# hbell99/DirectVoxGO

Hardware: AMD Instinct MI355X
Metric: train rays/sec (8192-ray batch, 160^3 grid) (higher is better)
Workload: dtype f32

## Files before the change

### directvoxgo_amd/csrc/common.h

```cpp
#pragma once
#include <hip/hip_runtime.h>
#include <stdint.h>

#include "../../include/dvgo_hip.h"

#define DVGO_WAVE 64
#define DVGO_BLOCK 256

#define DVGO_LAUNCH_CHECK()                                   \
  do {                                                        \
    hipError_t e__ = hipGetLastError();                       \
    if (e__ != hipSuccess) return (int)e__;                   \
  } while (0)

#define DVGO_HIP_TRY(expr)                                    \
  do {                                                        \
    hipError_t e__ = (expr);                                  \
    if (e__ != hipSuccess) return (int)e__;                   \
  } while (0)

static inline int dvgo_blocks(int64_t work, int per_block) {
  return (int)((work + per_block - 1) / per_block);
}

static inline bool dvgo_fits(int64_t work) { return work >= 0 && work < ((int64_t)1 << 31); }

__device__ __forceinline__ float dvgo_relu(float z) { return __builtin_elementwise_maximum(z, 0.0f); }
__device__ __forceinline__ unsigned int dvgo_relu_bit(float r) { return __float_as_uint(r) != 0u ? 1u : 0u; }

struct TriSetup {
  int i0, j0, k0;
  float wx0, wx1, wy0, wy1, wz0, wz1;
  float gx, gy, gz;
};

__device__ __forceinline__ float dvgo_src_index(float p, float mn, float mx, int size) {
  const float u = (p - mn) / (mx - mn);
  const float c = u * 2.0f - 1.0f;
  return ((c + 1.0f) / 2.0f) * (float)(size - 1);
}

__device__ __forceinline__ TriSetup dvgo_tri_from_g(float gx, float gy, float gz) {
  TriSetup t;
  const float fx = floorf(gx), fy = floorf(gy), fz = floorf(gz);
  t.i0 = (int)fx; t.j0 = (int)fy; t.k0 = (int)fz;
  t.wx0 = (fx + 1.0f) - gx; t.wx1 = gx - fx;
  t.wy0 = (fy + 1.0f) - gy; t.wy1 = gy - fy;
  t.wz0 = (fz + 1.0f) - gz; t.wz1 = gz - fz;
  t.gx = gx; t.gy = gy; t.gz = gz;
  return t;
}

__device__ __forceinline__ TriSetup dvgo_tri_setup(float px, float py, float pz,
                                                   float mnx, float mny, float mnz,
                                                   float mxx, float mxy, float mxz,
                                                   int X, int Y, int Z) {
  const float gx = dvgo_src_index(px, mnx, mxx, X);
  const float gy = dvgo_src_index(py, mny, mxy, Y);
  const float gz = dvgo_src_index(pz, mnz, mxz, Z);
  return dvgo_tri_from_g(gx, gy, gz);
}
// ... 144 lines not shown
```

### directvoxgo_amd/csrc/loss.hip

```cpp
#include "common.h"

__device__ __forceinline__ float block_sum_256(float v, float* red) {
#pragma unroll
  for (int d = 32; d >= 1; d >>= 1) v += __shfl_xor(v, d);
  const int lane = threadIdx.x & 63, w = threadIdx.x >> 6;
  if (lane == 0) red[w] = v;
  __syncthreads();
  const float t = red[0] + red[1] + red[2] + red[3];
  __syncthreads();
  return t;
}

__global__ void __launch_bounds__(256)
loss_rays_kernel(const float* __restrict__ rgb_marched, const float* __restrict__ alphainv_last,
                 const float* __restrict__ target, int64_t N, float inv_n_global, float w_main, float w_ent,
                 float* __restrict__ g_marched, float* __restrict__ g_last, float* __restrict__ loss_out) {
  __shared__ float red[4];
  const int64_t r = (int64_t)blockIdx.x * blockDim.x + threadIdx.x;
  float l = 0.0f;
  if (r < N) {
    float se = 0.0f;
#pragma unroll
    for (int c = 0; c < 3; ++c) {
      const float d = rgb_marched[3 * r + c] - target[3 * r + c];
// ... 5 lines not shown
      const float x = alphainv_last[r];
      const float p = fminf(fmaxf(x, 1e-6f), 1.0f - 1e-6f);
      const float lp = logf(p), lq = logf(1.0f - p);
      l += w_ent * (-(p * lp + (1.0f - p) * lq)) * inv_n_global;
      const bool inside = (x >= 1e-6f) && (x <= 1.0f - 1e-6f);
      g_last[r] = inside ? w_ent * (lq - lp) * inv_n_global : 0.0f;
    } else {
      g_last[r] = 0.0f;
    }
  }
  const float t = block_sum_256(l, red);
  if (threadIdx.x == 0) atomicAdd(loss_out, t);
}

__global__ void __launch_bounds__(256)
loss_samples_kernel(const float* __restrict__ raw_rgb, const float* __restrict__ weights,
                    const int64_t* __restrict__ ray_id, const float* __restrict__ target, int64_t M_cap,
                    const int64_t* __restrict__ m_dev,
                    float inv_n_global, float w_per, float* __restrict__ g_raw_rgb, float* __restrict__ loss_out) {
  const int64_t M = m_dev ? (*m_dev < M_cap ? *m_dev : M_cap) : M_cap;
  __shared__ float red[4];
  float l = 0.0f;
  for (int64_t i = (int64_t)blockIdx.x * blockDim.x + threadIdx.x; i < M; i += (int64_t)gridDim.x * blockDim.x) {
    const int64_t r = ray_id[i];
    const float w = weights[i];
    float se = 0.0f;
#pragma unroll
    for (int c = 0; c < 3; ++c) {
      const float d = raw_rgb[3 * i + c] - target[3 * r + c];
      se = fmaf(d, d, se);
      g_raw_rgb[3 * i + c] = 2.0f * w_per * w * d * inv_n_global;
    }
    l += w_per * w * se * inv_n_global;
  }
  const float t = block_sum_256(l, red);
  if (threadIdx.x == 0) atomicAdd(loss_out, t);
}

__global__ void __launch_bounds__(256)
viewdir_embed_kernel(const float* __restrict__ viewdirs, const float* __restrict__ freq, int F, int64_t N,
                     float* __restrict__ emb) {
  const int E = 3 + 6 * F;
  const int64_t t = (int64_t)blockIdx.x * blockDim.x + threadIdx.x;
  if (t >= N * E) return;
  const int64_t r = t / E;
  const int e = (int)(t - r * E);
  float v;
  if (e < 3) v = viewdirs[3 * r + e];
  else {
    const int q = (e - 3) % (3 * F);
    const float a = viewdirs[3 * r + q / F] * freq[q % F];
    v = (e - 3 < 3 * F) ? sinf(a) : cosf(a);
  }
  emb[t] = v;
}

#define DVGO_MT_MAX 16
struct AdamMulti {
  float* p[DVGO_MT_MAX];
  const float* g[DVGO_MT_MAX];
  float* m[DVGO_MT_MAX];
  float* v[DVGO_MT_MAX];
  int64_t start[DVGO_MT_MAX + 1];
  int n;
};
__global__ void __launch_bounds__(256)
// ... 44 lines not shown
  for (int k = n_tensors; k <= 8; ++k) A.start[k] = tot;
  if (tot == 0) return 0;
  if (!dvgo_fits(tot)) return DVGO_ERANGE;
  copy_multi_kernel<<<dvgo_blocks(tot, 256), 256, 0, (hipStream_t)stream>>>(A);
  DVGO_LAUNCH_CHECK();
  return 0;
}

int dvgo_loss_fwd_bwd(const float* rgb_marched, const float* alphainv_last, const float* target, int64_t N,
                      const float* raw_rgb, const float* weights, const int64_t* ray_id, int64_t M, const int64_t* m_dev,
                      int64_t n_rays_global, float w_main, float w_ent, float w_per, float* g_marched,
                      float* g_last, float* g_raw_rgb, float* loss_out, void* stream) {
  if (N < 0 || M < 0 || n_rays_global <= 0) return DVGO_EINVAL;
  if (!loss_out) return DVGO_EINVAL;
  hipStream_t s = (hipStream_t)stream;
  DVGO_HIP_TRY(hipMemsetAsync(loss_out, 0, sizeof(float), s));
  const float inv = 1.0f / (float)n_rays_global;
  if (N > 0) {
    if (!rgb_marched || !alphainv_last || !target || !g_marched || !g_last) return DVGO_EINVAL;
    loss_rays_kernel<<<dvgo_blocks(N, 256), 256, 0, s>>>(rgb_marched, alphainv_last, target, N, inv, w_main, w_ent,
                                                         g_marched, g_last, loss_out);
    DVGO_LAUNCH_CHECK();
  }
  if (M > 0 && w_per > 0.0f) {
    if (!raw_rgb || !weights || !ray_id || !g_raw_rgb) return DVGO_EINVAL;
    const int64_t nb = dvgo_blocks(M, 256);
    loss_samples_kernel<<<(int)(nb < 256 ? nb : (M >= (1 << 20) ? 1024 : 256)), 256, 0, s>>>(raw_rgb, weights, ray_id, target, M, m_dev, inv, w_per,
                                                            g_raw_rgb, loss_out);
    DVGO_LAUNCH_CHECK();
  }
  return 0;
}

int dvgo_viewdir_embed(const float* viewdirs, const float* freq, int n_freq, int64_t N, float* emb, void* stream) {
  if (N < 0 || n_freq < 0) return DVGO_EINVAL;
  if (N == 0) return 0;
  if (!viewdirs || !emb || (n_freq > 0 && !freq)) return DVGO_EINVAL;
  const int64_t total = N * (3 + 6 * n_freq);
  if (!dvgo_fits(total)) return DVGO_ERANGE;
  viewdir_embed_kernel<<<dvgo_blocks(total, 256), 256, 0, (hipStream_t)stream>>>(viewdirs, freq, n_freq, N, emb);
  DVGO_LAUNCH_CHECK();
  return 0;
}

int dvgo_adam_upd_multi(float* const* params, const float* const* grads, float* const* exp_avg,
                        float* const* exp_avg_sq, const int64_t* numel, int n_tensors, float step_size, float beta1,
                        float beta2, float eps, const float* step_size_dev, void* stream) {
  if (n_tensors < 0 || n_tensors > DVGO_MT_MAX) return DVGO_EINVAL;
  if (n_tensors == 0) return 0;
  if (!params || !grads || !exp_avg || !exp_avg_sq || !numel) return DVGO_EINVAL;
  AdamMulti A;
  A.n = n_tensors;
  int64_t tot = 0;
  for (int k = 0; k < n_tensors; ++k) {
    if (numel[k] < 0 || (numel[k] > 0 && (!params[k] || !grads[k] || !exp_avg[k] || !exp_avg_sq[k]))) return DVGO_EINVAL;
    A.p[k] = params[k]; A.g[k] = grads[k]; A.m[k] = exp_avg[k]; A.v[k] = exp_avg_sq[k];
    A.start[k] = tot;
    tot += numel[k];
  }
  for (int k = n_tensors; k <= DVGO_MT_MAX; ++k) A.start[k] = tot;
  if (tot == 0) return 0;
  adam_multi_kernel<<<dvgo_blocks(tot, 256), 256, 0, (hipStream_t)stream>>>(A, step_size, step_size_dev, beta1, beta2, eps);
  DVGO_LAUNCH_CHECK();
  return 0;
}

// ... 2 lines not shown
```

### directvoxgo_amd/csrc/shade_x3.hip

```cpp
#include "common.h"
#include "x3.h"

#ifndef X3_THREADS
#define X3_THREADS 512
#endif
#define X3_WAVES (X3_THREADS / 64)
#ifndef X3_BWD_THREADS
#define X3_BWD_THREADS 512
#endif
#define X3_BWD_WAVES (X3_BWD_THREADS / 64)
#define X3_STAGE_ROWS 16
#define X3_STAGE_STRIDE 36

__device__ __forceinline__ int x3_acc_feature(int t, int r, int h) { return 32 * t + (r & 3) + 8 * (r >> 2) + 4 * h; }

__device__ __forceinline__ void x3_split1(float v, unsigned short& s0, unsigned short& s1, unsigned short& s2) {
  const unsigned int h = x3_pack(v, 0.f) & 0xffffu;
  const float r = v - __uint_as_float(h << 16);
  const unsigned int m = x3_pack(r, 0.f) & 0xffffu;
  const float q = r - __uint_as_float(m << 16);
  s0 = (unsigned short)h; s1 = (unsigned short)m; s2 = (unsigned short)(x3_pack(q, 0.f) & 0xffffu);
}

template <int WIDTH, int KS1>
// ... 52 lines not shown
  for (int i = tid; i < T * KS1 * 64 * 8; i += nt) {
    const int j = i & 7, l = (i >> 3) & 63, s = (i >> 9) % KS1, t = (i >> 9) / KS1;
    const int k = 16 * s + 8 * (l >> 5) + j;
    const float v = (k < D_in) ? W1[(32 * t + (l & 31)) * D_in + k] : 0.0f;
    unsigned short p0, p1, p2;
    x3_split1(v, p0, p1, p2);
    reinterpret_cast<unsigned short*>(&L.w1s[t][s][0][l])[j] = p0;
    reinterpret_cast<unsigned short*>(&L.w1s[t][s][1][l])[j] = p1;
    reinterpret_cast<unsigned short*>(&L.w1s[t][s][2][l])[j] = p2;
  }
  for (int i = tid; i < T * 2 * T * 64 * 8; i += nt) {
    const int j = i & 7, l = (i >> 3) & 63, ks = (i >> 9) % (2 * T), t2 = (i >> 9) / (2 * T);
    const int k = 16 * ks + 8 * (j >> 2) + 4 * (l >> 5) + (j & 3);
    const float v = W2[(32 * t2 + (l & 31)) * WIDTH + k];
    unsigned short p0, p1, p2;
    x3_split1(v, p0, p1, p2);
    reinterpret_cast<unsigned short*>(&L.w2s[t2][ks][0][l])[j] = p0;
    reinterpret_cast<unsigned short*>(&L.w2s[t2][ks][1][l])[j] = p1;
    reinterpret_cast<unsigned short*>(&L.w2s[t2][ks][2][l])[j] = p2;
  }
  for (int i = tid; i < 3 * 2 * T * 16; i += nt) {
    const int tr = i % (T * 16), h = (i / (T * 16)) & 1, c = i / (2 * T * 16);
    (&L.w3p[0][0][0])[i] = W3[c * WIDTH + x3_acc_feature(tr >> 4, tr & 15, h)];
  }
  for (int i = tid; i < 2 * T * 16; i += nt) {
    const int tr = i % (T * 16), h = i / (T * 16);
    const int f = x3_acc_feature(tr >> 4, tr & 15, h);
    (&L.b1p[0][0])[i] = b1[f];
    (&L.b2p[0][0])[i] = b2[f];
  }
  if (tid < 4) L.b3[tid] = tid < 3 ? b3[tid] : 0.0f;
}

template <int WIDTH, int KS1, bool DIFFUSE>
__global__ void __launch_bounds__(X3_THREADS)
shade_fwd_x3_kernel(const float* __restrict__ feat, int C, int c_view0, int n_view, const float* __restrict__ emb, int E,
                    const int64_t* __restrict__ ray_id, int64_t M_cap, const int64_t* __restrict__ m_dev,
                    const void* __restrict__ image, float* __restrict__ rgb,
                    float* __restrict__ H1, float* __restrict__ H2, unsigned long long* __restrict__ masks, int experiment) {
  const int64_t M = m_dev ? (*m_dev < M_cap ? *m_dev : M_cap) : M_cap;
  constexpr int T = WIDTH / 32;
  __shared__ __attribute__((aligned(16))) X3Lds<WIDTH, KS1> L;
  x3_copy_image<X3Img<WIDTH, KS1>>(&L, image);
  __syncthreads();
  const int lane = threadIdx.x & 63, h = lane >> 5;
  float* stage = L.stage[threadIdx.x >> 6];
  const bool train = H1 != nullptr;
  const int64_t n_tiles = (M + 31) / 32;
  const int64_t gw = (int64_t)blockIdx.x * (blockDim.x >> 6) + (threadIdx.x >> 6);
  const int64_t nw = (int64_t)gridDim.x * (blockDim.x >> 6);
  const int d_in = n_view + E;
  const int64_t last = M > 0 ? M - 1 : 0;
  auto row_of = [&](int64_t tile) { const int64_t r = tile * 32 + (lane & 31); return r < M ? r : last; };
  float xin[KS1][8];
  auto load_inputs = [&](int64_t tile, int64_t rid) {
    const float* fr = feat + row_of(tile) * C + c_view0;
    const float* er = emb + rid * E - n_view;
#pragma unroll
    for (int s = 0; s < KS1; ++s)
#pragma unroll
      for (int j = 0; j < 8; ++j) {
        const int k = 16 * s + 8 * h + j;
        const int kc = k < d_in ? k : d_in - 1;
        xin[s][j] = *((kc < n_view) ? fr + kc : er + kc);
      }
  };
  int64_t rid_n = 0;
  if (gw < n_tiles) { load_inputs(gw, ray_id[row_of(gw)]); rid_n = ray_id[row_of(gw + nw)]; }
  for (int64_t tile = gw; tile < n_tiles; tile += nw) {
    const int64_t row = tile * 32 + (lane & 31);
    const bool valid = row < M;
    const int rows_valid = (int)(M - tile * 32 < 32 ? M - tile * 32 : 32);
    u32x4 x3[KS1][3];
#pragma unroll
    for (int s = 0; s < KS1; ++s) {
      float v[8];
#pragma unroll
      for (int j = 0; j < 8; ++j) v[j] = (16 * s + 8 * h + j) < d_in ? xin[s][j] : 0.0f;
      x3_split8(v, x3[s][0], x3[s][1], x3[s][2]);
    }
    load_inputs(tile + nw, rid_n);
    rid_n = ray_id[row_of(tile + 2 * nw)];
    u32x4 h3[2 * T][3];
    unsigned long long mask1 = 0ull;
#pragma unroll
    for (int t = 0; t < T; ++t) {
      f32x16 acc;
#pragma unroll
      for (int r = 0; r < 16; ++r) acc[r] = L.b1p[h][t * 16 + r];
#pragma unroll
      for (int s = 0; s < KS1; ++s)
        x3_mfma6(acc, L.w1s[t][s][0][lane], L.w1s[t][s][1][lane], L.w1s[t][s][2][lane], x3[s][0], x3[s][1], x3[s][2]);
#pragma unroll
      for (int r = 0; r < 16; ++r) acc[r] = dvgo_relu(acc[r]);
      if (train) {
        unsigned int bits = 0u;
#pragma unroll
        for (int r = 0; r < 16; ++r) bits |= dvgo_relu_bit(acc[r]) << r;
        mask1 |= (unsigned long long)bits << (16 * t);
        if (!(experiment & 512)) x3_store_tile(stage, acc, H1 + tile * 32 * WIDTH + 32 * t, WIDTH, lane, rows_valid);
      }
#pragma unroll
      for (int s2 = 0; s2 < 2; ++s2) {
        float v[8];
#pragma unroll
        for (int j = 0; j < 8; ++j) v[j] = acc[8 * s2 + j];
        x3_split8(v, h3[2 * t + s2][0], h3[2 * t + s2][1], h3[2 * t + s2][2]);
      }
      __builtin_amdgcn_sched_barrier(0);
    }
    float p[3] = {0.0f, 0.0f, 0.0f};
    unsigned long long mask2 = 0ull;
#pragma unroll 1
    for (int t2 = 0; t2 < T; ++t2) {
      f32x16 acc2;
#pragma unroll
      for (int r = 0; r < 16; ++r) acc2[r] = L.b2p[h][t2 * 16 + r];
      u32x4 a[2][3];
#pragma unroll
      for (int q = 0; q < 3; ++q) a[0][q] = L.w2s[t2][0][q][lane];
#pragma unroll
      for (int ks = 0; ks < 2 * T; ++ks) {
        if (ks + 1 < 2 * T) {
#pragma unroll
          for (int q = 0; q < 3; ++q) a[(ks + 1) & 1][q] = L.w2s[t2][ks + 1][q][lane];
        }
        x3_mfma6(acc2, a[ks & 1][0], a[ks & 1][1], a[ks & 1][2], h3[ks][0], h3[ks][1], h3[ks][2]);
        __builtin_amdgcn_sched_barrier(0);
      }
#pragma unroll
      for (int r = 0; r < 16; ++r) acc2[r] = dvgo_relu(acc2[r]);
      if (train) {
        unsigned int bits = 0u;
#pragma unroll
        for (int r = 0; r < 16; ++r) bits |= dvgo_relu_bit(acc2[r]) << r;
        mask2 |= (unsigned long long)bits << (16 * t2);
        if (!(experiment & 512)) x3_store_tile(stage, acc2, H2 + tile * 32 * WIDTH + 32 * t2, WIDTH, lane, rows_valid);
      }
#pragma unroll
      for (int c = 0; c < 3; ++c) {
#pragma unroll
        for (int r = 0; r < 16; ++r) p[c] = fmaf(L.w3p[c][h][t2 * 16 + r], acc2[r], p[c]);
      }
    }
    float z[3];
#pragma unroll
    for (int c = 0; c < 3; ++c) z[c] = p[c] + __shfl_xor(p[c], 32) + L.b3[c];
    if (valid) {
      if (h == 0) {
#pragma unroll
        for (int c = 0; c < 3; ++c) {
          const float zz = DIFFUSE ? z[c] + feat[row * C + c] : z[c];
          rgb[row * 3 + c] = 1.0f / (1.0f + expf(-zz));
        }
      }
      if (train) {
        masks[(row * 2 + 0) * 2 + h] = mask1;
        masks[(row * 2 + 1) * 2 + h] = mask2;
      }
    }
  }
}

template <int WIDTH>
struct X3BwdImg {
  static constexpr int T = WIDTH / 32;
  u32x4 w2t[T][2 * T][3][64];
  u32x4 w1t[2 * T][3][64];
// ... 853 lines not shown
}

extern "C" {

int64_t dvgo_shade_scratch_bytes(int width) {
  if (width == 128) return (int64_t)sizeof(X3Img<128, 3>) > (int64_t)sizeof(X3BwdImg<128>) ? sizeof(X3Img<128, 3>) : sizeof(X3BwdImg<128>);
  if (width == 64) return (int64_t)sizeof(X3Img<64, 3>) > (int64_t)sizeof(X3BwdImg<64>) ? sizeof(X3Img<64, 3>) : sizeof(X3BwdImg<64>);
  return 0;
}

int dvgo_shade_fwd_x3(const float* feat, int C, const float* emb, int E, const int64_t* ray_id, int64_t M, const int64_t* m_dev,
                      const float* W1, const float* b1, const float* W2, const float* b2, const float* W3,
                      const float* b3, int width, int d_in, int diffuse, float* rgb, float* H1, float* H2,
                      uint64_t* masks, void* scratch, void* scratch_bwd, int experiment, void* stream) {
  if (M < 0 || C <= 0 || E < 0) return DVGO_EINVAL;
  if (M == 0) return 0;
  if (!feat || !emb || !ray_id || !W1 || !b1 || !W2 || !b2 || !W3 || !b3 || !rgb || !scratch) return DVGO_EINVAL;
  if ((H1 == nullptr) != (H2 == nullptr) || (H1 == nullptr) != (masks == nullptr)) return DVGO_EINVAL;
  const int c_view0 = diffuse ? 3 : 0;
  const int n_view = C - c_view0;
  if (n_view < 0 || d_in != n_view + E) return DVGO_EINVAL;
  if ((width != 128 && width != 64) || d_in > 48) return DVGO_ERANGE;
  hipStream_t s = (hipStream_t)stream;
  const int64_t n_tiles = (M + 31) / 32;
  const int64_t cap = 256;
  const int blocks = (int)((n_tiles + X3_WAVES - 1) / X3_WAVES < cap ? (n_tiles + X3_WAVES - 1) / X3_WAVES : cap);
#define DVGO_SHADE_X3(W, KS, DIFF)                                                                                       \
  do {                                                                                                                   \
    x3_prep_fwd_kernel<W, KS><<<scratch_bwd ? 64 : 32, 256, 0, s>>>((X3Img<W, KS>*)scratch, (X3BwdImg<W>*)scratch_bwd, W1, b1, W2, b2, W3, b3, d_in); \
    shade_fwd_x3_kernel<W, KS, DIFF><<<blocks, X3_THREADS, 0, s>>>(feat, C, c_view0, n_view, emb, E, ray_id, M, m_dev, scratch, rgb, \
                                                                    H1, H2, (unsigned long long*)masks, experiment);     \
  } while (0)
  if (width == 128) {
    if (diffuse) DVGO_SHADE_X3(128, 3, true); else DVGO_SHADE_X3(128, 3, false);
  } else {
    if (d_in <= 16) { if (diffuse) DVGO_SHADE_X3(64, 1, true); else DVGO_SHADE_X3(64, 1, false); }
    else            { if (diffuse) DVGO_SHADE_X3(64, 3, true); else DVGO_SHADE_X3(64, 3, false); }
  }
#undef DVGO_SHADE_X3
  DVGO_LAUNCH_CHECK();
  return 0;
}

int dvgo_shade_bwd_x3(const float* g_rgb, const float* rgb, const uint64_t* masks, int64_t M, const int64_t* m_dev,
                      const float* W1, const float* W2, const float* W3, int width, int d_in, int C, int diffuse,
                      float* g_feat, float* G1, float* gz, void* scratch, int prebuilt, void* stream) {
  if (M < 0 || C <= 0) return DVGO_EINVAL;
  if (M == 0) return 0;
  if (!g_rgb || !rgb || !masks || !W1 || !W2 || !W3 || !g_feat || !G1 || !gz || !scratch) return DVGO_EINVAL;
  const int c_view0 = diffuse ? 3 : 0;
  const int n_view = C - c_view0;
  if ((width != 128 && width != 64) || n_view < 0 || n_view > 32 || d_in < n_view) return DVGO_ERANGE;
  hipStream_t s = (hipStream_t)stream;
  const int64_t n_tiles = (M + 31) / 32;
  const int64_t cap = 256;
  const int blocks = (int)((n_tiles + X3_BWD_WAVES - 1) / X3_BWD_WAVES < cap ? (n_tiles + X3_BWD_WAVES - 1) / X3_BWD_WAVES : cap);
#define DVGO_SHADE_BWD_X3(W, DIFF)                                                                                        \
  do {                                                                                                                    \
    if (!prebuilt) x3_prep_bwd_kernel<W><<<32, 256, 0, s>>>((X3BwdImg<W>*)scratch, W1, W2, W3, d_in);                   \
    shade_bwd_x3_kernel<W, DIFF><<<blocks, X3_BWD_THREADS, 0, s>>>(g_rgb, rgb, (const unsigned long long*)masks, M, m_dev, scratch, C, \
                                                                c_view0, n_view, g_feat, G1, gz);                         \
  } while (0)
  if (width == 128) { if (diffuse) DVGO_SHADE_BWD_X3(128, true); else DVGO_SHADE_BWD_X3(128, false); }
  else              { if (diffuse) DVGO_SHADE_BWD_X3(64, true); else DVGO_SHADE_BWD_X3(64, false); }
#undef DVGO_SHADE_BWD_X3
  DVGO_LAUNCH_CHECK();
  return 0;
// ... 37 lines not shown
```

### directvoxgo_amd/fused.py

```python
import math

import torch

from . import _lib as L
from ._lib import check_f32, check_input, f3, stream_of
from .ops import _grid_geom

_MAX_STRIDE_SCRATCH_BYTES = 4 << 30


class MarchConfig:

    def __init__(self, xyz_min, xyz_max, stepdist, act_shift, interval, fast_color_thres, near, far,
                 mask=None, xyz2ijk_scale=None, xyz2ijk_shift=None, ndc_samples=0):
        self.xyz_min_t, self.xyz_max_t = xyz_min, xyz_max
        self.xyz_min_h, self.xyz_max_h = f3(xyz_min), f3(xyz_max)
        self.stepdist = float(stepdist)
        self.act_shift = float(act_shift)
        self.interval = float(interval)
        self.thres = float(fast_color_thres)
        self.near, self.far = float(near), float(far)
        self.ndc_samples = int(ndc_samples)
        if self.ndc_samples > 0:
            self.stepdist = -float(self.ndc_samples - 1)
# ... 345 lines not shown
    mask = cfg.mask
    with L.device_of(rays_o):
        st = stream_of(rays_o)
        L.call('dvgo_sample_pts_prepare', rays_o, rays_d, cfg.xyz_min_t, cfg.xyz_max_t, cfg.near, cfg.far, cfg.stepdist, N,
               t_min, t_max, n_steps, None, start, dirs, st)
        L.call('dvgo_march_hit', start, dirs, n_steps, N, cfg.xyz_min_h, cfg.xyz_max_h, cfg.stepdist, mask, mask.shape[0],
               mask.shape[1], mask.shape[2], cfg.scale_h, cfg.shift_h, hit, st)
    return hit


def fused_march(density, k0, rays_o, rays_d, cfg, capacity=False, positions=False):
    if torch.is_grad_enabled() and (rays_o.requires_grad or rays_d.requires_grad) and (positions or cfg.ndc_samples > 0):
        raise NotImplementedError('fused_march: rays that require grad are not differentiated through '
                                  + ('the positional-encoding head\'s position input' if positions else 'NDC sampling'))
    return _FusedMarch.apply(density, k0, rays_o.contiguous(), rays_d.contiguous(), cfg, capacity, positions)


class _Composite(torch.autograd.Function):
    @staticmethod
    def forward(ctx, weights, rgb, alphainv_last, ray_id, off3, bg, m_dev=None):
        N = alphainv_last.shape[0]
        rgb = rgb.contiguous()
        weights = weights.contiguous()
        last = alphainv_last.contiguous()
        out = torch.empty((N, 3), dtype=torch.float32, device=weights.device)
        with L.device_of(weights):
            L.call('dvgo_march_composite', weights, rgb, None, off3, N, last, float(bg), out, None, stream_of(weights))
        ctx.save_for_backward(weights, rgb, ray_id)
        ctx.bg = float(bg)
        ctx.N = N
        ctx.m_dev = m_dev
        ctx.rgb_ptr, ctx.last_ptr = rgb.data_ptr(), last.data_ptr()
        ctx.extra = None
        return out

    @staticmethod
    @torch.autograd.function.once_differentiable
    def backward(ctx, g):
        weights, rgb, ray_id = ctx.saved_tensors
        g = g.contiguous()
        want_rgb, want_last = ctx.needs_input_grad[1], ctx.needs_input_grad[2]

        def bwd(gw, grgb, glast, accumulate):
            with L.device_of(weights):
                L.call('dvgo_march_composite_bwd', g, weights, rgb, ray_id, weights.shape[0], ctx.m_dev, ctx.N, ctx.bg, gw,
                       grgb, glast, accumulate, stream_of(weights))

        gw = torch.empty_like(weights) if ctx.needs_input_grad[0] else None
        (grgb, glast), accumulate = (ctx.extra, 1) if ctx.extra is not None else ((None, None), 0)
        ctx.extra = None
        g2 = torch.empty_like(rgb) if grgb is None and want_rgb else None
        l2 = torch.empty(ctx.N, dtype=torch.float32, device=g.device) if glast is None and want_last else None
        if not accumulate:
            bwd(gw, g2, l2, 0)
        else:
            if g2 is not None or l2 is not None:
                bwd(None, g2, l2, 0)
            bwd(gw, grgb, glast, 1)
        return gw, (grgb if grgb is not None else g2), (glast if glast is not None else l2), None, None, None, None


def composite(weights, rgb, alphainv_last, ray_id, off3, bg, m_dev=None):
    return _Composite.apply(weights, rgb, alphainv_last, ray_id, off3, bg, m_dev)


@torch.no_grad()
def composite_depth(weights, step_id, off3, n_rays):
    dev = weights.device
    dummy_rgb = torch.zeros((weights.shape[0], 3), dtype=torch.float32, device=dev)
    zeros = torch.zeros(n_rays, dtype=torch.float32, device=dev)
    out = torch.empty((n_rays, 3), dtype=torch.float32, device=dev)
# ... 6 lines not shown
```

### directvoxgo_amd/train.py

```python
import contextlib
import ctypes
from typing import NamedTuple

import torch
import torch.distributed as dist
import torch.nn as nn

from . import _lib as L
from .dp import GridReducer, flat_view
from .masked_adam import MaskedAdam
from .fused import brick_union, grid_rows_capture, split_grid_rows
from .shade import defer_wgrad


COARSE_TRAIN = dict(
    N_iters=5000, N_rand=8192, lrate_density=1e-1, lrate_k0=1e-1, lrate_rgbnet=1e-3, lrate_decay=20,
    pervoxel_lr=True, weight_main=1.0, weight_entropy_last=0.01, weight_rgbper=0.1,
    tv_every=1, tv_after=0, tv_before=0, tv_dense_before=0, weight_tv_density=0.0, weight_tv_k0=0.0,
    pg_scale=[], skip_zero_grad_fields=[])
FINE_TRAIN = dict(COARSE_TRAIN, N_iters=20000, pervoxel_lr=False, weight_entropy_last=0.001, weight_rgbper=0.01,
                  pg_scale=[1000, 2000, 3000, 4000], skip_zero_grad_fields=['density', 'k0'])


PLANE_REG_KEYS = ('weight_tv_planes', 'weight_tv_lines', 'weight_l1_lines')
# ... 17 lines not shown
            if isinstance(param, nn.Module):
                param = param.parameters()
            groups.append({'params': param, 'lr': lr, 'skip_zero_grad': name in cfg_train['skip_zero_grad_fields']})
        elif not isinstance(param, dict):
            param.requires_grad = False
    return MaskedAdam(groups)


def render_loss(render_result, target, n_rays_global, cfg_train):
    d = render_result['rgb_marched'] - target
    loss = cfg_train['weight_main'] * d.pow(2).sum() / (3 * n_rays_global)
    if cfg_train['weight_entropy_last'] > 0:
        pout = render_result['alphainv_last'].clamp(1e-6, 1 - 1e-6)
        ent = -(pout * torch.log(pout) + (1 - pout) * torch.log(1 - pout)).sum() / n_rays_global
        loss = loss + cfg_train['weight_entropy_last'] * ent
    if cfg_train['weight_rgbper'] > 0:
        rgbper = (render_result['raw_rgb'] - target[render_result['ray_id']]).pow(2).sum(-1)
        loss = loss + cfg_train['weight_rgbper'] * ((rgbper * render_result['weights'].detach()).sum() / n_rays_global)
    dist_loss = distortion_term(render_result, n_rays_global, cfg_train)
    return loss if dist_loss is None else loss + dist_loss


def distortion_term(render_result, n_rays_global, cfg_train):
    w = cfg_train.get('weight_distortion', 0)
    if not (w > 0 and 's' in render_result):
        return None
    from .distortion import distortion_loss
    return w * distortion_loss(render_result['weights'], render_result['s'], render_result['n_max'],
                               render_result['ray_id'], n_rays_global)


class _FusedLoss(torch.autograd.Function):
    unit_grad = False

    @staticmethod
    def forward(ctx, rgb_marched, alphainv_last, raw_rgb, weights, ray_id, target, n_global, w_main, w_ent, w_per, m_dev=None):
        N, M = rgb_marched.shape[0], raw_rgb.shape[0]
        dev = rgb_marched.device
        rgb_marched, alphainv_last, raw_rgb = rgb_marched.contiguous(), alphainv_last.contiguous(), raw_rgb.contiguous()
        g_marched = torch.empty_like(rgb_marched)
        g_last = torch.empty_like(alphainv_last)
        g_raw = torch.empty_like(raw_rgb) if w_per > 0 else None
        loss = torch.empty((), dtype=torch.float32, device=dev)
        with L.device_of(rgb_marched):
            L.call('dvgo_loss_fwd_bwd', rgb_marched, alphainv_last, target.contiguous(), N, raw_rgb, weights.contiguous(), ray_id,
                   M, m_dev, int(n_global), w_main, w_ent, w_per, g_marched, g_last, g_raw, loss, L.stream_of(rgb_marched))
        ctx.save_for_backward(g_marched, g_last, g_raw if g_raw is not None else g_last)
        ctx.has_raw = g_raw is not None
        fn = rgb_marched.grad_fn
        ctx.partner = None
        if (fn is not None and getattr(fn, 'rgb_ptr', None) == raw_rgb.data_ptr() and getattr(fn, 'last_ptr', None) ==
                alphainv_last.data_ptr() and raw_rgb.requires_grad and alphainv_last.requires_grad):
            ctx.partner = fn
        return loss

    @staticmethod
    @torch.autograd.function.once_differentiable
    def backward(ctx, go):
        g_marched, g_last, g_raw = ctx.saved_tensors
        unit = _FusedLoss.unit_grad
        gm = g_marched if unit else g_marched * go
        gl = g_last if unit else g_last * go
        gr = (g_raw if unit else g_raw * go) if ctx.has_raw else None
        if ctx.partner is not None:
            ctx.partner.extra = (gr, gl)
            ctx.partner = None
            return (gm, None, None, None, None, None, None, None, None, None, None)
        return (gm, gl, gr, None, None, None, None, None, None, None, None)


def fused_render_loss(render_result, target, n_rays_global, cfg_train):
    return _FusedLoss.apply(render_result['rgb_marched'], render_result['alphainv_last'], render_result['raw_rgb'],
                            render_result['weights'].detach(), render_result['ray_id'], target, n_rays_global,
                            float(cfg_train['weight_main']), float(cfg_train['weight_entropy_last']),
                            float(cfg_train['weight_rgbper']), render_result.get('n_samples'))


class _Plan(NamedTuple):
    path: str
    tv: bool
    keep_count: bool


class TrainStep:

    OVERLAP_MIN_SAMPLES = 600000

    def __init__(self, model, cfg_train, render_kwargs, optimizer=None, process_group=None, fused_loss=True,
                 overlap_wgrad=True, touched_reduce=True, rows_adam=True, track_mse=False, shard_grids=True, sync_free=False):
        self.model = model
        self.sync_free = sync_free
        self._m3_seen = None
        self._m3_pin, self._m3_event = None, None
# ... 129 lines not shown
    def _tv_weighted(self):
        return bool(self.cfg['weight_tv_density'] > 0 or self.cfg['weight_tv_k0'] > 0 or self.plane_reg_on)

    def _plan(self, rays_o, global_step):
        cfg, model, opt = self.cfg, self.model, self.optimizer
        tv = cfg['tv_after'] < global_step < cfg['tv_before'] and global_step % cfg['tv_every'] == 0 and self._tv_weighted()
        density, k0 = getattr(model, 'density', None), getattr(model, 'k0', None)
        own = (self.rows_adam and not tv and not self.k0_idle and not self.contracted and isinstance(opt, MaskedAdam)
               and isinstance(density, nn.Parameter) and isinstance(k0, nn.Parameter) and density.is_cuda)
        fuse_adam = own and opt.can_fuse_grid_step(density, k0)
        if self.dp is not None:
            path = 'tiles' if (fuse_adam and self.brick_sparse and getattr(model, 'fused', False)) else 'dense'
        else:
            path = 'fused' if fuse_adam else 'rows' if (own and opt.can_step_grid_rows(density, k0)) else 'dense'
        return _Plan(path, tv, bool(self.sync_free and self.fused_loss and rays_o.is_cuda
                                    and hasattr(model, 'can_keep_count_on_device') and model.can_keep_count_on_device()))

    def _decay_lr(self):
        for group in self.optimizer.param_groups:
            group['lr'] = group['lr'] * self.decay_factor

    def _eager(self, rays_o, rays_d, viewdirs, target, global_step):
        cfg, model, opt, dp = self.cfg, self.model, self.optimizer, self.dp
        if isinstance(opt, MaskedAdam) and opt.hyper_dev is not None and not self._capturing:
            opt.hyper_begin(model.density, model.k0)
        plan = self._plan(rays_o, global_step)
        n_global = rays_o.shape[0] * self.world
        density, k0 = getattr(model, 'density', None), getattr(model, 'k0', None)
        extra = {'_capacity': True} if plan.keep_count else {}
        with (brick_union(dp.pg, dp.BRICK_SPARSE_MAX) if plan.path == 'tiles' else contextlib.nullcontext()) as bu:
            res = model(rays_o, rays_d, viewdirs, global_step=global_step, **self.render_kwargs, **extra)
            opt.zero_grad(set_to_none=True)
            loss_fn = fused_render_loss if (self.fused_loss and res['rgb_marched'].is_cuda) else render_loss
            loss = loss_fn(res, target, n_global, cfg)
            dist_loss = distortion_term(res, n_global, cfg) if loss_fn is fused_render_loss else None
            if dist_loss is not None:
                loss = loss + dist_loss
            if self.track_mse:
                self.last_mse = cfg['weight_main'] * (res['rgb_marched'].detach() - target).pow(2).sum() / (3 * n_global)
            path = 'dense' if (plan.path == 'tiles' and not bu.sparse) else plan.path
            if path == 'tiles':
                dp.whole_grid_update_ahead()
            self.last_fused_adam = path in ('fused', 'tiles')
            rows = (grid_rows_capture(density, k0, adam=(lambda: opt.grid_step_args(density, k0)) if self.last_fused_adam else None)
                    if path != 'dense' else contextlib.nullcontext())
            n_samples = self._sample_count(res)
            side = self.overlap_wgrad and dp is None and n_samples >= self.OVERLAP_MIN_SAMPLES
            with defer_wgrad(side_stream=side) as deferred, rows as cap:
                _FusedLoss.unit_grad = True
                try:
                    loss.backward()
                finally:
                    _FusedLoss.unit_grad = False
        outcome = 'dense' if cap is None else 'stepped' if cap.stepped else 'rows' if cap.G is not None else 'dense'
        if outcome == 'stepped':
            assert density.grad is None and k0.grad is None
        elif outcome == 'rows':
            if density.grad is None and k0.grad is None:
                opt.step_grid_rows(density, k0, cap.G)
            else:
                gd, gk = split_grid_rows(cap.G, density, k0)
                density.grad = gd if density.grad is None else density.grad + gd
                k0.grad = gk if k0.grad is None else k0.grad + gk
            cap.G = None
        if dp is None:
            deferred.flush()
            self.last_mode = 'single'
# ... 26 lines not shown
```

### include/dvgo_hip.h

```cpp
#ifndef DVGO_HIP_H
#define DVGO_HIP_H

#include <stdint.h>

#ifdef __cplusplus
extern "C" {
#endif

#define DVGO_EINVAL (-1)
#define DVGO_ERANGE (-2)

#define DVGO_ABI_VERSION 11
int dvgo_abi_version(void);

#define DVGO_TUNE_FEAT_BWD    0
#define DVGO_TUNE_DENSITY_BWD 1
#define DVGO_TUNE_DENSITY_FWD 2
#define DVGO_TUNE_GATHER      3
#define DVGO_TUNE_EXPERIMENT  4
#define DVGO_TUNE_COUNT       8
int dvgo_set_tuning(int key, int value);

int dvgo_infer_t_minmax(const float* rays_o, const float* rays_d,
                        const float* xyz_min, const float* xyz_max,
// ... 193 lines not shown
int dvgo_shade_pe_fwd(const float* pts, const float* freq, int P, const float* emb, int E, const int64_t* ray_id, int64_t M,
                      const float* W1, const float* b1, const float* W2, const float* b2, const float* W3, const float* b3,
                      int width, int d_in, float* rgb, float* H1, float* H2, uint64_t* masks, void* stream);
int dvgo_shade_pe_bwd(const float* g_rgb, const float* rgb, const uint64_t* masks, int64_t M, const float* W2,
                      const float* W3, int width, float* G1, float* gz, void* stream);
int64_t dvgo_shade_pe_record_size(int width, int d_in);
int dvgo_shade_pe_wgrad(const float* G1, const float* gz, const uint64_t* masks, const float* W3, const float* H1,
                        const float* H2, const float* pts, const float* freq, int P, const float* emb, int E,
                        const int64_t* ray_id, int64_t M, int width, int d_in, int n_parts, float* part, float* total,
                        void* stream);

int dvgo_adam_upd(float* param, const float* grad, float* exp_avg, float* exp_avg_sq,
                  const float* perlr , int64_t n, float step_size,
                  float beta1, float beta2, float eps, int mode, void* stream);

int dvgo_adam_rows(const float* G, int64_t n_vox, int row_stride, int C,
                   float* p_k0, float* m_k0, float* v_k0, float step_size_k0, int mode_k0,
                   float* p_density, float* m_density, float* v_density, float step_size_density, int mode_density,
                   float beta1, float beta2, float eps, void* stream);

int dvgo_total_variation_add_grad(const float* param, float* grad, float wx, float wy, float wz,
                                  int64_t C, int64_t sz_i, int64_t sz_j, int64_t sz_k,
                                  int64_t sC, int64_t sI, int64_t sJ, int64_t sK,
                                  int dense_mode, void* stream);
int dvgo_total_variation_add_grad_slab(const float* param, float* grad, float wx, float wy, float wz,
                                       int64_t C, int64_t sz_i, int64_t sz_j, int64_t sz_k, int64_t sC,
                                       int64_t sI, int64_t sJ, int64_t sK, int dense_mode, int64_t i_lo, int64_t i_hi,
                                       void* stream);

int dvgo_loss_fwd_bwd(const float* rgb_marched, const float* alphainv_last, const float* target, int64_t N,
                      const float* raw_rgb, const float* weights, const int64_t* ray_id, int64_t M, const int64_t* m_dev,
                      int64_t n_rays_global, float w_main, float w_ent, float w_per,
                      float* g_marched, float* g_last, float* g_raw_rgb, float* loss_out, void* stream);
int dvgo_copy_multi(void* const* dst, const void* const* src, const int64_t* n_dwords, int n_tensors, void* stream);
int dvgo_viewdir_embed(const float* viewdirs, const float* freq, int n_freq, int64_t N, float* emb, void* stream);
int dvgo_adam_upd_multi(float* const* params, const float* const* grads, float* const* exp_avg,
                        float* const* exp_avg_sq, const int64_t* numel, int n_tensors, float step_size,
                        float beta1, float beta2, float eps,
                        const float* step_size_dev , void* stream);

int64_t dvgo_image_metrics_workspace_bytes(int64_t n, int H, int W, int filter_size);
int dvgo_image_metrics(const float* img0, const float* img1, int64_t n, int H, int W, const double* taps, int filter_size,
                       double c1, double c2, double* ssim_sum, double* sse, float* ssim_map,
                       void* workspace, int64_t workspace_bytes, void* stream);

int dvgo_mesh_field(const float* density, int X, int Y, int Z, const uint8_t* mask, int MX, int MY, int MZ,
                    const float* mask_scale, const float* mask_shift, int Rx, int Ry, int Rz, const float* g0,
                    const float* gs, const float* box_min, const float* spacing, int copy, float iso, float* field,
                    void* stream);
int dvgo_mesh_count(const float* field, int Px, int Py, int Pz, float iso, uint8_t* edge_mask, uint32_t* partials,
                    uint32_t* bases, void* stream);
int dvgo_mesh_emit(const float* field, const uint8_t* edge_mask, const uint32_t* bases, int Px, int Py, int Pz,
                   float iso, const float* box_min, const float* spacing, int64_t n_verts, int64_t n_faces,
                   float* verts, float* normals, int32_t* faces, void* stream);

int dvgo_contract_count(const float* rays_o, const float* rays_d, int64_t n_rays, const float* center,
                        const float* radius, const float* t_tab, int n_max, float bg_len, int l2, float thres,
                        const uint8_t* mask, int mi, int mj, int mk, const float* mask_scale,
                        const float* mask_shift, int32_t* counts, void* stream);
int dvgo_contract_emit(const float* rays_o, const float* rays_d, int64_t n_rays, const float* center,
                       const float* radius, const float* t_tab, int n_max, float bg_len, int l2, float thres,
                       const uint8_t* mask, int mi, int mj, int mk, const float* mask_scale, const float* mask_shift,
                       const int64_t* offsets, float* q, int64_t* ray_id, int64_t* step_id, float* t,
                       void* stream);
int dvgo_distortion_fwd_bwd(const float* w, const float* s, const int64_t* ray_id, int64_t m, int64_t n_rays,
                            int64_t n_norm, int n_max, float* grad, double* partials, unsigned int* ticket,
// ... 78 lines not shown
```

Measured before the change: 3.145 million.

## Fuse loss and compositing backward into one glue kernel; specialize shade input loads

Adds a loss_glue_kernel that computes the loss together with the alpha-compositing backward (gradients for raw rgb, weights and the last alpha) in one pass. The compositing autograd node then returns the precomputed gradients instead of running its own backward kernel. The path is enabled only while capturing. Separately, the shade forward kernel gets a compile-time specialization for 12 view channels and a 27-wide embedding to simplify input address selection, and ReLU mask bits now use an integer min instruction. The aim is to cut kernel launches and intermediate gradient traffic, at the cost of more intricate autograd coupling between the loss and render functions.

```diff
diff --git a/directvoxgo_amd/csrc/common.h b/directvoxgo_amd/csrc/common.h
--- a/directvoxgo_amd/csrc/common.h
+++ b/directvoxgo_amd/csrc/common.h
@@ -27,6 +27,11 @@
 
 __device__ __forceinline__ float dvgo_relu(float z) { return __builtin_elementwise_maximum(z, 0.0f); }
 __device__ __forceinline__ unsigned int dvgo_relu_bit(float r) { return __float_as_uint(r) != 0u ? 1u : 0u; }
+__device__ __forceinline__ unsigned int dvgo_relu_bit_int(float r) {
+  unsigned int b;
+  asm("v_min_u32 %0, 1, %1" : "=v"(b) : "v"(r));
+  return b;
+}
 
 struct TriSetup {
   int i0, j0, k0;
diff --git a/directvoxgo_amd/csrc/loss.hip b/directvoxgo_amd/csrc/loss.hip
--- a/directvoxgo_amd/csrc/loss.hip
+++ b/directvoxgo_amd/csrc/loss.hip
@@ -61,6 +61,76 @@
       g_raw_rgb[3 * i + c] = 2.0f * w_per * w * d * inv_n_global;
     }
     l += w_per * w * se * inv_n_global;
+  }
+  const float t = block_sum_256(l, red);
+  if (threadIdx.x == 0) atomicAdd(loss_out, t);
+}
+
+__global__ void __launch_bounds__(256)
+loss_glue_kernel(const float* __restrict__ rgb_marched, const float* __restrict__ alphainv_last,
+                 const float* __restrict__ target, int64_t N, const float* __restrict__ raw_rgb,
+                 const float* __restrict__ weights, const int64_t* __restrict__ ray_id, int64_t M_cap,
+                 const int64_t* __restrict__ m_dev, float inv_n_global, float w_main, float w_ent, float w_per, float bg,
+                 float* __restrict__ g_last, float* __restrict__ g_rgb, float* __restrict__ g_w,
+                 float* __restrict__ loss_out) {
+  const int64_t M = m_dev ? (*m_dev < M_cap ? *m_dev : M_cap) : M_cap;
+  __shared__ float red[4];
+  const int64_t t0 = (int64_t)blockIdx.x * blockDim.x + threadIdx.x, nt = (int64_t)gridDim.x * blockDim.x;
+  float l = 0.0f;
+  for (int64_t r = t0; r < N; r += nt) {
+    float se = 0.0f, gm[3];
+#pragma unroll
+    for (int c = 0; c < 3; ++c) {
+      const float d = rgb_marched[3 * r + c] - target[3 * r + c];
+      se = fmaf(d, d, se);
+      gm[c] = 2.0f * w_main * d * inv_n_global * (1.0f / 3.0f);
+    }
+    float lr = w_main * se * inv_n_global * (1.0f / 3.0f), gl = 0.0f;
+    if (w_ent > 0.0f) {
+      const float x = alphainv_last[r];
+      const float p = fminf(fmaxf(x, 1e-6f), 1.0f - 1e-6f);
+      const float lp = logf(p), lq = logf(1.0f - p);
+      lr += w_ent * (-(p * lp + (1.0f - p) * lq)) * inv_n_global;
+      const bool inside = (x >= 1e-6f) && (x <= 1.0f - 1e-6f);
+      gl = inside ? w_ent * (lq - lp) * inv_n_global : 0.0f;
+    }
+    l += lr;
+    if (g_last) g_last[r] = (gm[0] + gm[1] + gm[2]) * bg + gl;
+  }
+  for (int64_t i0 = t0; i0 < M; i0 += 4 * nt) {
+    int64_t r[4];
+    float w[4], x[4][3], tg[4][3], rm[4][3];
+#pragma unroll
+    for (int u = 0; u < 4; ++u) {
+      const int64_t i = i0 + u * nt < M ? i0 + u * nt : M - 1;
+      r[u] = ray_id[i];
+      w[u] = weights[i];
+#pragma unroll
+      for (int c = 0; c < 3; ++c) x[u][c] = raw_rgb[3 * i + c];
+    }
+#pragma unroll
+    for (int u = 0; u < 4; ++u)
+#pragma unroll
+      for (int c = 0; c < 3; ++c) { tg[u][c] = target[3 * r[u] + c]; rm[u][c] = rgb_marched[3 * r[u] + c]; }
+#pragma unroll
+    for (int u = 0; u < 4; ++u) {
+      const int64_t i = i0 + u * nt;
+      if (i >= M) break;
+      float gm[3], se = 0.0f;
+#pragma unroll
+      for (int c = 0; c < 3; ++c) {
+        gm[c] = 2.0f * w_main * (rm[u][c] - tg[u][c]) * inv_n_global * (1.0f / 3.0f);
+        if (w_per > 0.0f) {
+          const float d = x[u][c] - tg[u][c];
+          se = fmaf(d, d, se);
+          if (g_rgb) g_rgb[3 * i + c] = fmaf(gm[c], w[u], 2.0f * w_per * w[u] * d * inv_n_global);
+        } else if (g_rgb) {
+          g_rgb[3 * i + c] = gm[c] * w[u];
+        }
+      }
+      if (w_per > 0.0f) l += w_per * w[u] * se * inv_n_global;
+      if (g_w) g_w[i] = fmaf(gm[2], x[u][2], fmaf(gm[1], x[u][1], gm[0] * x[u][0]));
+    }
   }
   const float t = block_sum_256(l, red);
   if (threadIdx.x == 0) atomicAdd(loss_out, t);
@@ -171,6 +241,27 @@
   return 0;
 }
 
+int dvgo_loss_composite_bwd(const float* rgb_marched, const float* alphainv_last, const float* target, int64_t N,
+                            const float* raw_rgb, const float* weights, const int64_t* ray_id, int64_t M,
+                            const int64_t* m_dev, int64_t n_rays_global, float w_main, float w_ent, float w_per, float bg,
+                            float* g_last, float* g_rgb, float* g_w, float* loss_out, void* stream) {
+  if (N < 0 || M < 0 || n_rays_global <= 0) return DVGO_EINVAL;
+  if (!loss_out) return DVGO_EINVAL;
+  hipStream_t s = (hipStream_t)stream;
+  DVGO_HIP_TRY(hipMemsetAsync(loss_out, 0, sizeof(float), s));
+  if (N == 0 && M == 0) return 0;
+  if (N > 0 && (!rgb_marched || !alphainv_last || !target)) return DVGO_EINVAL;
+  if (M > 0 && (N == 0 || !raw_rgb || !weights || !ray_id)) return DVGO_EINVAL;
+  const int64_t threads = M > N ? M : N;
+  if (!dvgo_fits(threads)) return DVGO_ERANGE;
+  const int64_t nb = dvgo_blocks(threads, 256), cap = M >= (1 << 20) ? 1024 : 256;
+  loss_glue_kernel<<<(int)(nb < cap ? nb : cap), 256, 0, s>>>(rgb_marched, alphainv_last, target, N, raw_rgb, weights, ray_id, M,
+                                                              m_dev, 1.0f / (float)n_rays_global, w_main, w_ent, w_per, bg,
+                                                              g_last, g_rgb, g_w, loss_out);
+  DVGO_LAUNCH_CHECK();
+  return 0;
+}
+
 int dvgo_viewdir_embed(const float* viewdirs, const float* freq, int n_freq, int64_t N, float* emb, void* stream) {
   if (N < 0 || n_freq < 0) return DVGO_EINVAL;
   if (N == 0) return 0;
diff --git a/directvoxgo_amd/csrc/shade_x3.hip b/directvoxgo_amd/csrc/shade_x3.hip
--- a/directvoxgo_amd/csrc/shade_x3.hip
+++ b/directvoxgo_amd/csrc/shade_x3.hip
@@ -108,7 +108,7 @@
   if (tid < 4) L.b3[tid] = tid < 3 ? b3[tid] : 0.0f;
 }
 
-template <int WIDTH, int KS1, bool DIFFUSE>
+template <int WIDTH, int KS1, bool DIFFUSE, int NV = -1, int CV0 = 0, int EE = 0>
 __global__ void __launch_bounds__(X3_THREADS)
 shade_fwd_x3_kernel(const float* __restrict__ feat, int C, int c_view0, int n_view, const float* __restrict__ emb, int E,
                     const int64_t* __restrict__ ray_id, int64_t M_cap, const int64_t* __restrict__ m_dev,
@@ -125,21 +125,39 @@
   const int64_t n_tiles = (M + 31) / 32;
   const int64_t gw = (int64_t)blockIdx.x * (blockDim.x >> 6) + (threadIdx.x >> 6);
   const int64_t nw = (int64_t)gridDim.x * (blockDim.x >> 6);
-  const int d_in = n_view + E;
+  constexpr bool FIXED = NV >= 0;
+  const int d_in = FIXED ? NV + EE : n_view + E;
   const int64_t last = M > 0 ? M - 1 : 0;
   auto row_of = [&](int64_t tile) { const int64_t r = tile * 32 + (lane & 31); return r < M ? r : last; };
   float xin[KS1][8];
   auto load_inputs = [&](int64_t tile, int64_t rid) {
-    const float* fr = feat + row_of(tile) * C + c_view0;
-    const float* er = emb + rid * E - n_view;
-#pragma unroll
-    for (int s = 0; s < KS1; ++s)
-#pragma unroll
-      for (int j = 0; j < 8; ++j) {
-        const int k = 16 * s + 8 * h + j;
-        const int kc = k < d_in ? k : d_in - 1;
-        xin[s][j] = *((kc < n_view) ? fr + kc : er + kc);
-      }
+    if constexpr (FIXED) {
+      const float* f0 = feat + row_of(tile) * (CV0 + NV) + CV0;
+      const float* e0 = emb + rid * EE - NV;
+      const float* fh = f0 + 8 * h;
+      const float* eh = e0 + 8 * h;
+      const float* mh = h ? e0 + 8 : f0;
+#pragma unroll
+      for (int s = 0; s < KS1; ++s)
+#pragma unroll
+        for (int j = 0; j < 8; ++j) {
+          const int k0 = 16 * s + j, k1 = k0 + 8;
+          const int lo = k0 < NV ? 0 : k0 < NV + EE ? 1 : 2, hi = k1 < NV ? 0 : k1 < NV + EE ? 1 : 2;
+          xin[s][j] = (lo == 0 && hi == 0) ? fh[k0] : (lo == 0 && hi == 1) ? mh[k0] : (lo == 1 && hi == 1) ? eh[k0]
+                    : lo == 0 ? f0[k0] : lo == 1 ? e0[k0] : 0.0f;
+        }
+    } else {
+      const float* fr = feat + row_of(tile) * C + c_view0;
+      const float* er = emb + rid * E - n_view;
+#pragma unroll
+      for (int s = 0; s < KS1; ++s)
+#pragma unroll
+        for (int j = 0; j < 8; ++j) {
+          const int k = 16 * s + 8 * h + j;
+          const int kc = k < d_in ? k : d_in - 1;
+          xin[s][j] = *((kc < n_view) ? fr + kc : er + kc);
+        }
+    }
   };
   int64_t rid_n = 0;
   if (gw < n_tiles) { load_inputs(gw, ray_id[row_of(gw)]); rid_n = ray_id[row_of(gw + nw)]; }
@@ -172,7 +190,7 @@
       if (train) {
         unsigned int bits = 0u;
 #pragma unroll
-        for (int r = 0; r < 16; ++r) bits |= dvgo_relu_bit(acc[r]) << r;
+        for (int r = 0; r < 16; ++r) bits |= dvgo_relu_bit_int(acc[r]) << r;
         mask1 |= (unsigned long long)bits << (16 * t);
         if (!(experiment & 512)) x3_store_tile(stage, acc, H1 + tile * 32 * WIDTH + 32 * t, WIDTH, lane, rows_valid);
       }
@@ -209,7 +227,7 @@
       if (train) {
         unsigned int bits = 0u;
 #pragma unroll
-        for (int r = 0; r < 16; ++r) bits |= dvgo_relu_bit(acc2[r]) << r;
+        for (int r = 0; r < 16; ++r) bits |= dvgo_relu_bit_int(acc2[r]) << r;
         mask2 |= (unsigned long long)bits << (16 * t2);
         if (!(experiment & 512)) x3_store_tile(stage, acc2, H2 + tile * 32 * WIDTH + 32 * t2, WIDTH, lane, rows_valid);
       }
@@ -1129,7 +1147,12 @@
                                                                     H1, H2, (unsigned long long*)masks, experiment);     \
   } while (0)
   if (width == 128) {
-    if (diffuse) DVGO_SHADE_X3(128, 3, true); else DVGO_SHADE_X3(128, 3, false);
+    if (diffuse) DVGO_SHADE_X3(128, 3, true);
+    else if (n_view == 12 && E == 27 && !(experiment & 1024)) {
+      x3_prep_fwd_kernel<128, 3><<<scratch_bwd ? 64 : 32, 256, 0, s>>>((X3Img<128, 3>*)scratch, (X3BwdImg<128>*)scratch_bwd, W1, b1, W2, b2, W3, b3, d_in);
+      shade_fwd_x3_kernel<128, 3, false, 12, 0, 27><<<blocks, X3_THREADS, 0, s>>>(feat, C, c_view0, n_view, emb, E, ray_id, M, m_dev, scratch, rgb,
+                                                                                  H1, H2, (unsigned long long*)masks, experiment);
+    } else DVGO_SHADE_X3(128, 3, false);
   } else {
     if (d_in <= 16) { if (diffuse) DVGO_SHADE_X3(64, 1, true); else DVGO_SHADE_X3(64, 1, false); }
     else            { if (diffuse) DVGO_SHADE_X3(64, 3, true); else DVGO_SHADE_X3(64, 3, false); }
diff --git a/directvoxgo_amd/fused.py b/directvoxgo_amd/fused.py
--- a/directvoxgo_amd/fused.py
+++ b/directvoxgo_amd/fused.py
@@ -401,11 +401,20 @@
         ctx.m_dev = m_dev
         ctx.rgb_ptr, ctx.last_ptr = rgb.data_ptr(), last.data_ptr()
         ctx.extra = None
+        ctx.glue_key = (weights.data_ptr(), rgb.data_ptr(), last.data_ptr(), ray_id.data_ptr(),
+                        None if m_dev is None else m_dev.data_ptr())
+        ctx.done = None
+        ctx.set_materialize_grads(False)
         return out
 
     @staticmethod
     @torch.autograd.function.once_differentiable
     def backward(ctx, g):
+        if ctx.done is not None:
+            done, ctx.done = ctx.done, None
+            return (*done, None, None, None, None)
+        if g is None:
+            return (None,) * 7
         weights, rgb, ray_id = ctx.saved_tensors
         g = g.contiguous()
         want_rgb, want_last = ctx.needs_input_grad[1], ctx.needs_input_grad[2]
diff --git a/directvoxgo_amd/train.py b/directvoxgo_amd/train.py
--- a/directvoxgo_amd/train.py
+++ b/directvoxgo_amd/train.py
@@ -73,22 +73,37 @@
 
 class _FusedLoss(torch.autograd.Function):
     unit_grad = False
+    glue = False
 
     @staticmethod
     def forward(ctx, rgb_marched, alphainv_last, raw_rgb, weights, ray_id, target, n_global, w_main, w_ent, w_per, m_dev=None):
         N, M = rgb_marched.shape[0], raw_rgb.shape[0]
         dev = rgb_marched.device
         rgb_marched, alphainv_last, raw_rgb = rgb_marched.contiguous(), alphainv_last.contiguous(), raw_rgb.contiguous()
+        weights, target = weights.contiguous(), target.contiguous()
+        fn = rgb_marched.grad_fn
+        ctx.glued = False
+        if (_FusedLoss.glue and fn is not None and raw_rgb.requires_grad and alphainv_last.requires_grad and
+                getattr(fn, 'glue_key', None) == (weights.data_ptr(), raw_rgb.data_ptr(), alphainv_last.data_ptr(),
+                                                  ray_id.data_ptr(), None if m_dev is None else m_dev.data_ptr())):
+            g_w = torch.empty_like(weights) if fn.needs_input_grad[0] else None
+            g_rgb, g_last = torch.empty_like(raw_rgb), torch.empty_like(alphainv_last)
+            loss = torch.empty((), dtype=torch.float32, device=dev)
+            with L.device_of(rgb_marched):
+                L.call('dvgo_loss_composite_bwd', rgb_marched, alphainv_last, target, N, raw_rgb, weights, ray_id, M, m_dev,
+                       int(n_global), w_main, w_ent, w_per, fn.bg, g_last, g_rgb, g_w, loss, L.stream_of(rgb_marched))
+            ctx.save_for_backward(g_rgb, g_last, g_w if g_w is not None else g_last)
+            ctx.glued, ctx.has_w, ctx.partner = True, g_w is not None, fn
+            return loss
         g_marched = torch.empty_like(rgb_marched)
         g_last = torch.empty_like(alphainv_last)
         g_raw = torch.empty_like(raw_rgb) if w_per > 0 else None
         loss = torch.empty((), dtype=torch.float32, device=dev)
         with L.device_of(rgb_marched):
-            L.call('dvgo_loss_fwd_bwd', rgb_marched, alphainv_last, target.contiguous(), N, raw_rgb, weights.contiguous(), ray_id,
+            L.call('dvgo_loss_fwd_bwd', rgb_marched, alphainv_last, target, N, raw_rgb, weights, ray_id,
                    M, m_dev, int(n_global), w_main, w_ent, w_per, g_marched, g_last, g_raw, loss, L.stream_of(rgb_marched))
         ctx.save_for_backward(g_marched, g_last, g_raw if g_raw is not None else g_last)
         ctx.has_raw = g_raw is not None
-        fn = rgb_marched.grad_fn
         ctx.partner = None
         if (fn is not None and getattr(fn, 'rgb_ptr', None) == raw_rgb.data_ptr() and getattr(fn, 'last_ptr', None) ==
                 alphainv_last.data_ptr() and raw_rgb.requires_grad and alphainv_last.requires_grad):
@@ -98,8 +113,16 @@
     @staticmethod
     @torch.autograd.function.once_differentiable
     def backward(ctx, go):
+        unit = _FusedLoss.unit_grad
+        if ctx.glued:
+            g_rgb, g_last, g_w = ctx.saved_tensors
+            g_w = g_w if ctx.has_w else None
+            if not unit:
+                g_rgb, g_last, g_w = g_rgb * go, g_last * go, (g_w * go if g_w is not None else None)
+            ctx.partner.done = (g_w, g_rgb, g_last)
+            ctx.partner = None
+            return (None,) * 11
         g_marched, g_last, g_raw = ctx.saved_tensors
-        unit = _FusedLoss.unit_grad
         gm = g_marched if unit else g_marched * go
         gl = g_last if unit else g_last * go
         gr = (g_raw if unit else g_raw * go) if ctx.has_raw else None
@@ -295,7 +318,11 @@
             res = model(rays_o, rays_d, viewdirs, global_step=global_step, **self.render_kwargs, **extra)
             opt.zero_grad(set_to_none=True)
             loss_fn = fused_render_loss if (self.fused_loss and res['rgb_marched'].is_cuda) else render_loss
-            loss = loss_fn(res, target, n_global, cfg)
+            _FusedLoss.glue = self._capturing
+            try:
+                loss = loss_fn(res, target, n_global, cfg)
+            finally:
+                _FusedLoss.glue = False
             dist_loss = distortion_term(res, n_global, cfg) if loss_fn is fused_render_loss else None
             if dist_loss is not None:
                 loss = loss + dist_loss
diff --git a/include/dvgo_hip.h b/include/dvgo_hip.h
--- a/include/dvgo_hip.h
+++ b/include/dvgo_hip.h
@@ -249,6 +249,10 @@
                       const float* raw_rgb, const float* weights, const int64_t* ray_id, int64_t M, const int64_t* m_dev,
                       int64_t n_rays_global, float w_main, float w_ent, float w_per,
                       float* g_marched, float* g_last, float* g_raw_rgb, float* loss_out, void* stream);
+int dvgo_loss_composite_bwd(const float* rgb_marched, const float* alphainv_last, const float* target, int64_t N,
+                            const float* raw_rgb, const float* weights, const int64_t* ray_id, int64_t M,
+                            const int64_t* m_dev, int64_t n_rays_global, float w_main, float w_ent, float w_per, float bg,
+                            float* g_last, float* g_rgb, float* g_w, float* loss_out, void* stream);
 int dvgo_copy_multi(void* const* dst, const void* const* src, const int64_t* n_dwords, int n_tensors, void* stream);
 int dvgo_viewdir_embed(const float* viewdirs, const float* freq, int n_freq, int64_t N, float* emb, void* stream);
 int dvgo_adam_upd_multi(float* const* params, const float* const* grads, float* const* exp_avg,
```

Measured after the change: 3.190 million (median of 6 runs). +1.4%, better.
